# M2-TE/noetic-slam

Hardware: AMD Instinct MI355X
Metric: scans/sec TSDF integration (128x1024 pts, 5 cm voxel) (higher is better)
Workload: dtype f64+f32; 1 GPU; C1/M1 ouster_os1_128_1024x10_synthetic_5cm; global_batch=64, scans_per_gpu_batch=64, pipelined_batches=2, semantics=vdbfusion_f64, parallelism=single, front_end=two walks (k_count + k_place)

## Files before the change

noetic-slam_amd/csrc/tsdf_capi.cpp:

```cpp
#include <hip/hip_runtime.h>

#include <algorithm>
#include <array>
#include <atomic>
#include <cmath>
#include <cstdarg>
#include <cstddef>
#include <cstdio>
#include <cstdlib>
#include <cstring>
#include <numeric>
#include <chrono>
#include <condition_variable>
#include <functional>
#include <mutex>
#include <string>
#include <thread>
#include <utility>
#include <vector>

#include "../../include/tsdf_hip.h"
#include "../../include/tsdf_hip_deskew.h"
#include "../../include/tsdf_hip_columns.h"
#include "../../include/tsdf_hip_esdf.h"
// ... 181 lines not shown
    HipHandle() = default;
    HipHandle(const HipHandle&) = delete;
    HipHandle& operator=(const HipHandle&) = delete;
    ~HipHandle() { if (h) (void)KILL(h); }
    hipError_t create() { return MAKE(&h, FLAGS); }
    operator H() const { return h; }
};
using Event = HipHandle<hipEvent_t, hipEventCreateWithFlags, hipEventDisableTiming, hipEventDestroy>;
using Stream = HipHandle<hipStream_t, hipStreamCreateWithFlags, hipStreamNonBlocking, hipStreamDestroy>;


struct Capacity {
    uint64_t max_bricks = 0, cap = 0;
    uint32_t max_active = 0;
    DevBuf<uint64_t> keys, brick_keys;
    DevBuf<uint32_t> slots, touched, cell[2];
    DevBuf<float> sdf, weight;
    DevBuf<uint4> active[2], active_ord[2], cagg[2];
};

struct Lane {
    DevBuf<uint32_t> pair, blk_n, plan, spn, ord_hist, act;
    DevBuf<uint32_t> tile;
    DevBuf<uint4> blk, fb;
    DevBuf<uint2> smp;
    DevBuf<uint64_t> mg_ekey;
    DevBuf<uint32_t> mg_eidx, mg_bcnt, mg_bst, mg_bscan;
    DevBuf<float> mg_xyz, mg_w;
};

struct ScanRing {
    static constexpr int N = 16;
    PinBuf<ScanRec> host;
// ... 231 lines not shown
    if (lean) HIPCHK(c, hipEventRecord(c->ev_compact[par], st));
    if (prev && !lean) HIPCHK(c, hipStreamWaitEvent(st, c->ev_integ[par ^ 1], 0));
    if (D.n_blocks) {
        if (tm && c->plan.fused) tm->begin(KIND_INTEGRATE, st);
        if (small) {
            HIPCHK(c, launch_integrate_small(B, c->R, T, W, c->Pl, c->G, par, st, kt(KIND_INTEGRATE)));
        } else {
            Work Wi = W;
            Wi.active = W.active_ord;
            HIPCHK(c, launch_integrate(B, c->R, T, Wi, c->Pl, c->G, par, c->plan.fused, c->max_batch > 64, st,
                                       kt(KIND_INTEGRATE)));
        }
        if (tm && c->plan.fused) tm->end(KIND_INTEGRATE, st);
        c->ht.lap(HT_INTEGRATE);
    }
    HIPCHK(c, launch_finish(c->G, par, (uint32_t)c->batch_id, B, st));
    if (cross) {
        HIPCHK(c, hipEventRecord(ring.ev[slot], st));
        c->ev_integ[par] = ring.ev[slot];
    }
    if (c->can_grow) c->log.push_back({c->batch_id, d_xyz, D});
    for (int k = 0; k < 2; k++)
        if (d_xyz == c->stage2[k]) {
            c->stage_reader[k] = c->batch_id;
            HIPCHK(c, hipEventRecord(c->stage_ev[k], st));
        }
    c->ht.lap(HT_FINISH);
    c->ht.n++;
    c->batch_id++;
    c->n_batches++;
    c->n_scans += D.n_scans;
// ... 59 lines not shown

static int settle(tsdf_ctx* c) {
    const int rc = flush(c);
    return rc ? rc : join(c);
}


static int alloc_capacity(tsdf_ctx* c, uint64_t max_bricks, Capacity& K) {
    K = Capacity{};
    K.max_bricks = max_bricks;
    K.cap = next_pow2(2 * max_bricks);
    K.max_active = (uint32_t)std::min<uint64_t>(K.cap, c->plan.slots);
    const size_t cells = K.cap * c->plan.cell_stride * (c->plan.fused ? sizeof(uint64_t) : sizeof(uint32_t));
    hipError_t e = K.keys.alloc(K.cap);
    if (e == hipSuccess) e = K.slots.alloc(K.cap);
    if (e == hipSuccess) e = K.touched.alloc(K.cap);
    if (e == hipSuccess) e = K.brick_keys.alloc(max_bricks);
    if (e == hipSuccess) e = K.sdf.alloc(max_bricks * BRICK_VOX);
    if (e == hipSuccess) e = K.weight.alloc(max_bricks * BRICK_VOX);
    for (int q = 0; q < 2 && e == hipSuccess; q++) {
        e = K.cell[q].alloc_bytes(cells);
        if (e == hipSuccess) e = K.active[q].alloc(K.max_active);
        if (e == hipSuccess) e = K.active_ord[q].alloc(K.max_active);
        if (e == hipSuccess) e = K.cagg[q].alloc(compact_chunks(K.cap) * 2);
    }
    if (e != hipSuccess) {
        (void)hipGetLastError();
        return fail(c, TSDF_ENOMEM, "device allocation for %llu bricks failed",
                    (unsigned long long)max_bricks);
    }
    e = launch_fill_u64(K.keys, EMPTY_KEY, K.cap, c->stream);
    if (e == hipSuccess) e = launch_fill_u32(K.slots, UNASSIGNED, K.cap, c->stream);
    if (e == hipSuccess) e = hipMemsetAsync(K.touched, 0, K.cap * sizeof(uint32_t), c->stream);
    for (int q = 0; q < 2 && e == hipSuccess; q++) e = hipMemsetAsync(K.cell[q], 0, cells, c->stream);
    if (e != hipSuccess) return fail(c, TSDF_EHIP, "capacity init: %s", hipGetErrorString(e));
    return TSDF_OK;
}

static void set_views(tsdf_ctx* c) {
    const Capacity& K = c->K;
    c->T = Table{K.keys, K.slots, K.touched, K.cell[0], K.brick_keys, K.cap - 1,
                 (uint32_t)K.max_bricks, c->plan.cell_stride};
    c->Pl = Pool{K.sdf, K.weight};
    const uint64_t mg_cap = c->merged ? c->plan.batch_points : 0;
    for (int q = 0; q < 2; q++) {
        const Lane& L = c->lane[q];
        c->W2[q] = Work{L.pair, L.blk, L.blk_n, L.plan, L.fb, L.smp, K.active[q], K.active_ord[q],
                        L.ord_hist, K.cagg[q], L.act, L.spn, c->plan.maxp,
                        K.max_active, c->max_fb, c->max_smp, c->max_spn};
        c->mg[q] = MgBufs{L.mg_xyz, L.mg_w, mg_cap, L.mg_ekey, L.mg_eidx, L.mg_bcnt, L.mg_bst,
                          L.mg_bscan, mg_cap ? mg_buckets_max(mg_cap) : 0};
    }
}


struct GlobalsCheck { uint32_t pool_count, overflow, failed, retry, fail_id; };
static_assert(offsetof(Globals, pool_count) == 0 && offsetof(Globals, overflow) == 4 &&
              offsetof(Globals, failed) == 8 && offsetof(Globals, retry) == 12 &&
              offsetof(Globals, fail_id) == 16 && offsetof(Globals, ctr) < offsetof(Globals, tot_vox),
              "the host reads and clears Globals' head by these offsets");
static hipError_t globals_clear(uint32_t* first, int words) {
    const uint32_t z[3] = {0u, 0u, 0u};
    return hipMemcpy(first, z, 4 * words, hipMemcpyHostToDevice);
// ... 21 lines not shown
        if (e == hipSuccess)
            e = hipMemcpyAsync(K.brick_keys, c->T.brick_keys, valid * 8, hipMemcpyDeviceToDevice,
                               c->stream);
    }
    if (e == hipSuccess) e = launch_fill(K.sdf + valid * BRICK_VOX, c->R.bg, (nb - valid) * BRICK_VOX, c->stream);
    if (e == hipSuccess)
        e = hipMemsetAsync(K.weight + valid * BRICK_VOX, 0, (nb - valid) * BRICK_VOX * 4, c->stream);
    if (e == hipSuccess) e = hipStreamSynchronize(c->stream);
    if (e != hipSuccess) return fail(c, TSDF_EHIP, "grow: %s", hipGetErrorString(e));
    c->K = std::move(K);
    set_views(c);
    HIPCHK(c, launch_rehash(c->T, (uint32_t)valid, c->G, c->stream));
    const uint32_t pcv = (uint32_t)valid, retry = 1u;
    HIPCHK(c, hipMemsetAsync(c->G, 0, offsetof(Globals, tot_vox), c->stream));
    HIPCHK(c, hipMemcpyAsync(&c->G->pool_count, &pcv, 4, hipMemcpyHostToDevice, c->stream));
    HIPCHK(c, hipMemcpyAsync(&c->G->retry, &retry, 4, hipMemcpyHostToDevice, c->stream));
    HIPCHK(c, hipStreamSynchronize(c->stream));
    c->n_grows++;
    return TSDF_OK;
}

template <class T>
static int grow_list(tsdf_ctx* c, DevBuf<T> Lane::*list, uint32_t tsdf_ctx::*max, uint64_t limit,
                     size_t bytes, const char* what, bool counted) {
    const uint64_t n = std::min<uint64_t>(2ull * (c->*max), limit);
    if (n <= c->*max) return fail(c, TSDF_ENOMEM, "%s at its limit", what);
    DevBuf<T> f[2];
    hipError_t e = f[0].alloc_bytes(n * bytes);
    if (e == hipSuccess) e = f[1].alloc_bytes(n * bytes);
    if (e != hipSuccess) {
// ... 1740 lines not shown
            if (rc == TSDF_EHIP) return rc;
        }
    }
    Scratch tmp;
    int32_t* dc = nullptr;
    float *ds = nullptr, *dw = nullptr;
    uint32_t* dt = nullptr;
    HIPCHK(c, tmp.get(c, &dc, n * 3));
    HIPCHK(c, tmp.get(c, &ds, n * BRICK_VOX));
    HIPCHK(c, tmp.get(c, &dw, n * BRICK_VOX));
    HIPCHK(c, tmp.get(c, &dt, n));
    HIPCHK(c, hipMemcpyAsync(dc, coords, n * 12, hipMemcpyHostToDevice, c->stream));
    HIPCHK(c, hipMemcpyAsync(ds, sdf, n * BRICK_VOX * 4, hipMemcpyHostToDevice, c->stream));
    HIPCHK(c, hipMemcpyAsync(dw, weight, n * BRICK_VOX * 4, hipMemcpyHostToDevice, c->stream));
    HIPCHK(c, launch_import(c->T, c->Pl, dc, (uint32_t)n, ds, dw, dt, c->G, merge_cap(c), c->stream));
    HIPCHK(c, hipStreamSynchronize(c->stream));
    return tsdf_sync(c);
}

}


static int merge_ctx_state(tsdf_ctx* d, tsdf_ctx* c, const char* which) {
    if (c->p.n_sectors > 1)
        return fail(d, TSDF_EINVAL, "merge: the %s context holds one sector shard of the map "
                                    "(n_sectors > 1); merging a sharded field is not supported", which);
    if (c->brd_open)
        return fail(d, TSDF_EINVAL, "merge: a border reduce is open on the %s context: commit or "
                                    "abort it first (tsdf_border_commit_device)", which);
    return TSDF_OK;
// ... 73 lines not shown
    if (!apply || !st.touched_bricks) return TSDF_OK;

    const uint64_t need = n_dst + st.new_bricks;
    if (need > d->T.max_bricks) {
        if (!d->can_grow || (d->p.max_bricks_hard && need > d->p.max_bricks_hard) ||
            need > 0xFFFFFFEFull)
            return fail(d, TSDF_ENOMEM, "merge: %llu new bricks do not fit the pool (%llu of %llu "
                                        "bricks in use) and it cannot grow",
                        (unsigned long long)st.new_bricks, (unsigned long long)n_dst,
                        (unsigned long long)d->T.max_bricks);
        rc = grow_capacity(d, need);
        if (rc) return rc;
    }
    HIPCHK(d, launch_merge_apply(d->T, d->Pl, s->T, s->Pl, s->R, X, mode, min_weight, merge_cap(d),
                                 list, n_cand, flag, tslot, d->G, d->stream));
    HIPCHK(d, hipStreamSynchronize(d->stream));
    return tsdf_sync(d);
}

extern "C" {

int tsdf_merge_count(tsdf_ctx* dst, tsdf_ctx* src, const double pose[12], int32_t mode,
                     float min_weight, tsdf_merge_stats* out) {
    return merge_impl(dst, src, pose, mode, min_weight, out, false);
}

int tsdf_merge_transformed(tsdf_ctx* dst, tsdf_ctx* src, const double pose[12], int32_t mode,
                           float min_weight, tsdf_merge_stats* out) {
    return merge_impl(dst, src, pose, mode, min_weight, out, true);
}
// ... 32 lines not shown
                    M.new_count, M.n, M.n_moves);
    return TSDF_OK;
}

static int removal_compact(tsdf_ctx* c, const Removal& M) {
    if (!M.removed()) return TSDF_OK;
    const Capacity& K = c->K;
    const uint64_t at = (uint64_t)M.new_count * BRICK_VOX, freed = (uint64_t)M.removed() * BRICK_VOX;
    HIPCHK(c, launch_rm_move(c->T, c->Pl, M.rml, M.mover, M.n_moves, c->stream));
    HIPCHK(c, launch_fill(c->Pl.sdf + at, c->R.bg, freed, c->stream));
    HIPCHK(c, hipMemsetAsync(c->Pl.weight + at, 0, freed * sizeof(float), c->stream));
    HIPCHK(c, launch_fill_u64(K.keys, EMPTY_KEY, K.cap, c->stream));
    HIPCHK(c, launch_fill_u32(K.slots, UNASSIGNED, K.cap, c->stream));
    const size_t cells = K.cap * c->plan.cell_stride *
                         (c->plan.fused ? sizeof(uint64_t) : sizeof(uint32_t));
    HIPCHK(c, hipMemsetAsync(K.touched, 0, K.cap * sizeof(uint32_t), c->stream));
    for (int q = 0; q < 2; q++) HIPCHK(c, hipMemsetAsync(K.cell[q], 0, cells, c->stream));
    HIPCHK(c, launch_rehash(c->T, M.new_count, c->G, c->stream));
    HIPCHK(c, hipMemcpyAsync(&c->G->pool_count, &M.new_count, 4, hipMemcpyHostToDevice, c->stream));
    HIPCHK(c, hipStreamSynchronize(c->stream));
    return TSDF_OK;
}

static int removal_enter(tsdf_ctx* c, const int32_t* lo, const int32_t* hi, bool box, uint64_t* nb) {
    if (border_busy(c)) return TSDF_EINVAL;
    if (box) {
        if (!lo || !hi) return fail(c, TSDF_EINVAL, "null box");
        for (int a = 0; a < 3; a++)
            if (lo[a] > hi[a]) return fail(c, TSDF_EINVAL, "box: lo > hi");
    }
    return pool_bricks(c, nb);
}

extern "C" {
// ... 592 lines not shown
```

noetic-slam_amd/csrc/tsdf_device.h:

```cpp
#pragma once
#include <hip/hip_ext.h>
#include <hip/hip_runtime.h>
#include <stdint.h>

#include "os_headers.h"

namespace tsdf {

constexpr uint64_t EMPTY_KEY = ~0ull;
constexpr uint32_t UNASSIGNED = 0xFFFFFFFFu;
constexpr uint32_t INVALID_SLOT = 0xFFFFFFFEu;
constexpr uint32_t NO_PAIR = 0xFFFFFFFFu;
constexpr int BRICK_VOX = 512;
constexpr int BRICK_COORD_BIAS = 1 << 20;
constexpr int VOX_LIMIT = 1 << 23;
constexpr int MAX_DDA_STEPS = 1 << 20;
constexpr int MAX_BATCH = 512;
#ifndef TSDF_RPB
#define TSDF_RPB 1024
#endif
#ifndef TSDF_HCAP
#define TSDF_HCAP 2048
#endif
constexpr int RPB = TSDF_RPB;
// ... 76 lines not shown
struct BatchDesc {
    uint32_t n_scans;
    uint32_t n_blocks;
    ScanRec s[MAX_BATCH + 1];
};
struct BatchRef {
    uint32_t n_scans;
    uint32_t n_blocks;
    const ScanRec* __restrict__ s;
    const uint32_t* __restrict__ tile;
};

struct Table {
    uint64_t* keys;
    uint32_t* slots;
    uint32_t* touched;
    uint32_t* cell;
    uint64_t* brick_keys;
    uint64_t mask;
    uint32_t max_bricks;
    uint32_t cell_stride;
};

struct Pool {
    float* sdf;
    float* weight;
};

struct Work {
    uint32_t* pair;
    uint4* blk;
    uint32_t* blk_n;
    uint32_t* plan;
    uint4* fb;
    uint2* smp;
    uint4* active;
    uint4* active_ord;
    uint32_t* ord_hist;
    uint4* cagg;
    uint32_t* act;
    uint32_t* spn;
    uint32_t maxp;
    uint32_t max_active;
    uint32_t max_fb;
    uint32_t max_smp;
    uint32_t max_spn;
};

constexpr size_t smp_bytes(int sem) { return sem == 3 ? 12 : 8; }
template <int SEM>
__device__ __forceinline__ void smp_store(const Work& W, uint32_t i, float s, uint32_t tl, float w) {
    if constexpr (SEM == 3)
        reinterpret_cast<uint3*>(W.smp)[i] = make_uint3(__float_as_uint(s), tl, __float_as_uint(w));
    else
// ... 28 lines not shown
constexpr uint32_t METRIC_RING = 256;
struct BatchRecord {
    uint32_t batch_id, n_active, n_new, ovf;
    uint32_t committed, pool_count;
    uint32_t tiled;
    uint32_t pad;
    unsigned long long rays, pairs, vox, dirty;
};

struct Globals {
    uint32_t pool_count;
    uint32_t overflow;
    uint32_t failed;
    uint32_t retry;
    uint32_t fail_id;
    uint32_t pad[3];
    Counters ctr[2];
    unsigned long long tot_vox[8];
    unsigned long long tot_rays[8];
    unsigned long long tot_pairs[8];
    unsigned long long tot_dirty[8];
    Counters last;
    BatchRecord ring[METRIC_RING];
};

enum KernelKind {
    KIND_COUNT = 0, KIND_COMPACT = 1, KIND_PLACE = 2, KIND_INTEGRATE = 3,
    KIND_WALK = 4, KIND_SPANS = 5,
    KIND_N = 6
};

// ... 14 lines not shown
    virtual void begin(int kind, hipStream_t st) = 0;
    virtual void end(int kind, hipStream_t st) = 0;
    virtual ~KernelTimer() {}
};

hipError_t launch_count(const float* d_xyz, const BatchRef& D, const RayConst& R, const Table& T,
                        const Work& Wk, Globals* G, int parity, hipStream_t st, const KTime& kt = {},
                        bool wide = false, bool paired = false);
hipError_t launch_tile_detect(const float* d_xyz, const BatchRef& D, uint32_t* tile,
                              uint32_t force, hipStream_t st);
#ifndef TSDF_CMP_CHUNK
#define TSDF_CMP_CHUNK 1024
#endif
constexpr uint32_t CMP_CHUNK = TSDF_CMP_CHUNK;
inline uint64_t compact_chunks(uint64_t cap) { return (cap + CMP_CHUNK - 1) / CMP_CHUNK; }
hipError_t launch_sector_flags(const float* d_xyz, const BatchRef& D, const RayConst& R,
                               const Work& Wk, Globals* G, int parity, hipStream_t st);
hipError_t launch_compact(const BatchRef& D, const Table& T, const Work& Wk, Globals* G,
                          int parity, bool fused, hipStream_t st, const KTime& kt = {});
hipError_t launch_walk(const float* d_xyz, const BatchRef& D, const RayConst& R, const Table& T,
                       const Work& Wk, Globals* G, int parity, int nstep, hipStream_t st);
hipError_t launch_spans(const BatchRef& D, const RayConst& R, const Table& T, const Work& Wk,
                        Globals* G, int parity, int nstep, hipStream_t st);
hipError_t launch_place(const float* d_xyz, const BatchRef& D, const RayConst& R, const Table& T,
                        const Work& Wk, Globals* G, int parity, hipStream_t st, const KTime& kt = {});
hipError_t launch_finish(Globals* G, int parity, uint32_t batch_id, const BatchRef& D,
                         hipStream_t st);
hipError_t launch_pool_mark(Globals* G, int parity, hipStream_t st);
hipError_t launch_upload(const void* host_src, void* dst, uint32_t bytes,
                         unsigned long long* done, unsigned long long seq, hipStream_t st);
hipError_t launch_rehash(const Table& T, uint32_t n, Globals* G, hipStream_t st);
hipError_t launch_integrate_small(const BatchRef& D, const RayConst& R, const Table& T,
                                  const Work& Wk, const Pool& Pl, Globals* G, int parity,
                                  hipStream_t st, const KTime& kt = {});
hipError_t launch_integrate(const BatchRef& D, const RayConst& R, const Table& T, const Work& Wk,
                            const Pool& Pl, Globals* G, int parity, bool fused, bool big,
                            hipStream_t st, const KTime& kt = {});
hipError_t launch_query_dense(const Table& T, const Pool& Pl, const int64_t lo[3], const int dims[3],
                              float bg, float* d_sdf, float* d_w, hipStream_t st);
hipError_t launch_import(const Table& T, const Pool& Pl, const int32_t* d_coords, uint32_t n,
                         const float* d_sdf, const float* d_w, uint32_t* d_tidx, Globals* G,
                         float max_w, hipStream_t st);
hipError_t launch_fill(float* p, float v, uint64_t n, hipStream_t st);
// ... 127 lines not shown
```

noetic-slam_amd/csrc/tsdf_kernels.hip:

```cpp
#include <hip/hip_runtime.h>
#include <stdint.h>

#include <type_traits>

#include "tsdf_device.h"
#include "tsdf_ray.h"

namespace tsdf {


__device__ __forceinline__ uint32_t xcd_wedge(uint32_t p, uint32_t n, uint32_t G) {
    const uint32_t grp = 8u * G, g0 = p - p % grp;
    if (g0 + grp > n) return p;
    const uint32_t i = p - g0;
    return g0 + (i % 8u) * G + i / 8u;
}

__device__ __forceinline__ int lds_insert(unsigned long long* s_key, uint64_t key) {
    uint32_t hs = (uint32_t)(mix64(key) >> 40) & (HCAP - 1);
    for (int p = 0; p < LDS_PROBES; p++) {
        const unsigned long long k = s_key[hs];
        if (k == key) return (int)hs;
        if (k == EMPTY_KEY) {
            const unsigned long long old = atomicCAS(&s_key[hs], EMPTY_KEY, key);
// ... 454 lines not shown

constexpr int ORD_BLOCKS = 64;
constexpr int ORD_CLASSES = 32;

__device__ __forceinline__ uint32_t size_class(uint32_t n) {
    return (uint32_t)__clz(max(n, 1u));
}
__device__ __forceinline__ uint32_t ord_chunk_slice(uint32_t c, uint32_t nch) {
    return (uint32_t)(((uint64_t)c * ORD_BLOCKS) / nch);
}


constexpr int CMP_THREADS = 256;
constexpr int CMP_PER = CMP_CHUNK / CMP_THREADS;
constexpr int CMP_GROUP = 16;
constexpr int CMP_SCAN_THREADS = 1024;

template <int NT>
__device__ __forceinline__ uint32_t block_excl_scan(uint32_t x, uint32_t* s_w, uint32_t* total) {
    constexpr int NW = NT / 64;
    const int lane = threadIdx.x & 63, wid = threadIdx.x >> 6;
    const uint32_t v = wave_incl_scan(x);
    if (lane == 63) s_w[wid] = v;
    __syncthreads();
    uint32_t off = 0, tot = 0;
#pragma unroll
    for (int k = 0; k < NW; k++) {
        const uint32_t r = s_w[k];
        off += k < wid ? r : 0u;
        tot += r;
    }
    *total = tot;
    __syncthreads();
    return v - x + off;
}

__device__ __forceinline__ uint32_t compact_list(const Table& T, uint32_t chunk, uint32_t* s_h,
                                                 uint32_t* s_w, bool clear) {
    uint32_t hit[CMP_PER], cnt = 0;
#pragma unroll
    for (int j = 0; j < CMP_PER; j++) {
        const uint32_t h = chunk + threadIdx.x * CMP_PER + j;
        hit[j] = h <= T.mask && T.touched[h] != 0u ? 1u : 0u;
        cnt += hit[j];
    }
    uint32_t nh;
    uint32_t e = block_excl_scan<CMP_THREADS>(cnt, s_w, &nh);
#pragma unroll
    for (int j = 0; j < CMP_PER; j++) {
        if (hit[j]) {
            const uint32_t h = chunk + threadIdx.x * CMP_PER + j;
            s_h[e++] = h;
            if (clear) T.touched[h] = 0u;
        }
    }
    __syncthreads();
    return nh;
}

template <bool FUSED>
__device__ __forceinline__ uint32_t row_groups(uint32_t n_scans) {
    return FUSED ? (n_scans + 2) / 2 : (n_scans + 3) / 4;
}
template <bool FUSED>
__device__ __forceinline__ uint32_t group_count(const uint4& v) {
    return FUSED ? v.y + v.w : v.x + v.y + v.z + v.w;
}
template <bool FUSED>
__device__ __forceinline__ const uint4* cell_row(const Table& T, uint32_t h) {
// ... 1 lines not shown
                                                  (size_t)h * T.cell_stride)
                 : reinterpret_cast<const uint4*>(T.cell + (size_t)h * T.cell_stride);
}

template <bool FUSED>
__global__ __launch_bounds__(CMP_THREADS) void k_compact_sum(uint32_t n_scans, Table T, Work Wk) {
    __shared__ uint32_t s_w[CMP_THREADS / 64];
    __shared__ uint32_t s_h[CMP_CHUNK];
    __shared__ uint32_t s_acc[2];
    if (threadIdx.x == 0) {
        s_acc[0] = 0u;
        s_acc[1] = 0u;
    }
    __shared__ uint32_t s_cls[ORD_CLASSES];
    if (threadIdx.x < ORD_CLASSES) s_cls[threadIdx.x] = 0u;
    const uint32_t nh = compact_list(T, blockIdx.x * CMP_CHUNK, s_h, s_w, false);
    const uint32_t nq = row_groups<FUSED>(n_scans);
    const uint32_t grp = threadIdx.x / CMP_GROUP, li = threadIdx.x % CMP_GROUP;
    uint32_t samples = 0, nnew = 0;
    for (uint32_t k = grp; k < nh; k += CMP_THREADS / CMP_GROUP) {
        const uint32_t h = s_h[k];
        const uint4* cp = cell_row<FUSED>(T, h);
        uint32_t sum = 0;
        for (uint32_t q = li; q < nq; q += CMP_GROUP) sum += group_count<FUSED>(cp[q]);
        samples += sum;
#pragma unroll
        for (int d = CMP_GROUP / 2; d >= 1; d >>= 1) sum += __shfl_xor(sum, d, CMP_GROUP);
        if (li == 0) atomicAdd(&s_cls[size_class(sum)], 1u);
        if (li == 0 && T.slots[h] == UNASSIGNED) nnew++;
    }
    samples = wave_sum<uint32_t>(samples);
    nnew = wave_sum<uint32_t>(nnew);
    if ((threadIdx.x & 63) == 0) {
        if (samples) atomicAdd(&s_acc[0], samples);
        if (nnew) atomicAdd(&s_acc[1], nnew);
    }
    __syncthreads();
    if (threadIdx.x == 0) Wk.cagg[blockIdx.x] = make_uint4(nh, s_acc[0], s_acc[1], 0u);
    if (threadIdx.x < ORD_CLASSES && s_cls[threadIdx.x])
        atomicAdd(&Wk.ord_hist[ord_chunk_slice(blockIdx.x, gridDim.x) * ORD_CLASSES + threadIdx.x],
                  s_cls[threadIdx.x]);
}

__global__ __launch_bounds__(CMP_SCAN_THREADS) void k_compact_scan(uint32_t nch, Work Wk,
                                                                   Globals* G, int parity,
                                                                   int fused) {
    __shared__ uint32_t s_w[3][CMP_SCAN_THREADS / 64];
    __shared__ uint32_t s_carry[3];
    Counters* C = &G->ctr[parity];
    if (threadIdx.x == 0) {
        s_carry[0] = 0u;
        s_carry[1] = 0u;
        s_carry[2] = G->pool_count;
    }
    __syncthreads();
    constexpr int NWS = CMP_SCAN_THREADS / 64;
    const int lane = threadIdx.x & 63, wid = threadIdx.x >> 6;
    const uint32_t P = (nch + CMP_SCAN_THREADS - 1) / CMP_SCAN_THREADS;
    const uint32_t c0 = threadIdx.x * P;
    uint32_t sa = 0, sc = 0, sn = 0;
#pragma unroll 4
    for (uint32_t q = 0; q < P; q++) {
        const uint4 a = c0 + q < nch ? Wk.cagg[c0 + q] : make_uint4(0u, 0u, 0u, 0u);
        sa += a.x;
        sc += a.y;
        sn += a.z;
    }
    const uint32_t ia = wave_incl_scan(sa), ic = wave_incl_scan(sc), in = wave_incl_scan(sn);
    if (lane == 63) {
        s_w[0][wid] = ia;
        s_w[1][wid] = ic;
        s_w[2][wid] = in;
    }
    __syncthreads();
    uint32_t oa = s_carry[0], oc = s_carry[1], on = s_carry[2], ta = 0, tc = 0, tn = 0;
#pragma unroll
    for (int k = 0; k < NWS; k++) {
        const uint32_t xa = s_w[0][k], xc = s_w[1][k], xn = s_w[2][k];
        oa += k < wid ? xa : 0u;
        oc += k < wid ? xc : 0u;
        on += k < wid ? xn : 0u;
        ta += xa;
        tc += xc;
        tn += xn;
    }
    oa += ia - sa;
    oc += ic - sc;
    on += in - sn;
    for (uint32_t q = 0; q < P && c0 + q < nch; q++) {
        const uint4 a = Wk.cagg[c0 + q];
        Wk.cagg[nch + c0 + q] = make_uint4(oa, oc, on, 0u);
        oa += a.x;
        oc += a.y;
        on += a.z;
    }
    if (threadIdx.x == 0) {
        s_carry[0] += ta;
        s_carry[1] += tc;
        s_carry[2] += tn;
    }
    __syncthreads();
    static_assert(ORD_BLOCKS == 64 && ORD_CLASSES == 32 && CMP_SCAN_THREADS == 1024, "layout");
    {
        __shared__ uint32_t s_tot[ORD_CLASSES], s_cbase[ORD_CLASSES];
        const int lane = threadIdx.x & 63, w = threadIdx.x >> 6;
        uint32_t v[2], ex[2];
#pragma unroll
        for (int q = 0; q < 2; q++) {
            const int cls = w + 16 * q;
            v[q] = Wk.ord_hist[lane * ORD_CLASSES + cls];
            const uint32_t incl = wave_incl_scan(v[q]);
            ex[q] = incl - v[q];
            if (lane == 63) s_tot[cls] = incl;
            Wk.ord_hist[lane * ORD_CLASSES + cls] = 0u;
        }
        __syncthreads();
        if (w == 0) {
            const uint32_t t = lane < ORD_CLASSES ? s_tot[lane] : 0u;
            const uint32_t incl = wave_incl_scan(t);
            if (lane < ORD_CLASSES) s_cbase[lane] = incl - t;
        }
        __syncthreads();
#pragma unroll
        for (int q = 0; q < 2; q++) {
            const int cls = w + 16 * q;
            Wk.ord_hist[ORD_BLOCKS * ORD_CLASSES + lane * ORD_CLASSES + cls] = s_cbase[cls] + ex[q];
        }
    }
    if (threadIdx.x == 0) {
        C->n_active = s_carry[0];
        C->cursor = s_carry[1];
        C->n_new = s_carry[2] - G->pool_count;
        G->pool_count = s_carry[2];
        C->pool = s_carry[2];
        if (fused ? s_carry[1] > Wk.max_spn : s_carry[1] > Wk.max_smp)
            atomicOr(&C->ovf, fused ? OVF_SPN : OVF_SMP);
        if (s_carry[0] > Wk.max_active) atomicOr(&C->ovf, OVF_ACTIVE);
    }
}

template <bool FUSED>
__global__ __launch_bounds__(CMP_THREADS) void k_compact_write(uint32_t n_scans, uint32_t nch,
                                                               Table T, Work Wk, Globals* G,
                                                               int parity) {
    __shared__ uint32_t s_w[CMP_THREADS / 64];
    __shared__ uint32_t s_h[CMP_CHUNK];
    __shared__ uint32_t s_n[CMP_CHUNK];
    const uint32_t chunk = blockIdx.x * CMP_CHUNK;
    const uint32_t nh = compact_list(T, chunk, s_h, s_w, true);
    if (nh == 0) return;
    const uint32_t nq = row_groups<FUSED>(n_scans);
    const uint32_t grp = threadIdx.x / CMP_GROUP, li = threadIdx.x % CMP_GROUP;
    for (uint32_t k = grp; k < nh; k += CMP_THREADS / CMP_GROUP) {
        const uint4* cp = cell_row<FUSED>(T, s_h[k]);
        uint32_t sum = 0;
        for (uint32_t q = li; q < nq; q += CMP_GROUP) sum += group_count<FUSED>(cp[q]);
#pragma unroll
        for (int d = CMP_GROUP / 2; d >= 1; d >>= 1) sum += __shfl_xor(sum, d, CMP_GROUP);
        if (li == 0) s_n[k] = sum;
    }
    __syncthreads();
    const uint4 base = Wk.cagg[nch + blockIdx.x];
    uint32_t n[CMP_PER], isnew[CMP_PER], sn = 0, snew = 0;
#pragma unroll
    for (int j = 0; j < CMP_PER; j++) {
        const uint32_t k = threadIdx.x * CMP_PER + j;
        n[j] = k < nh ? s_n[k] : 0u;
        isnew[j] = k < nh && T.slots[s_h[k]] == UNASSIGNED ? 1u : 0u;
        sn += n[j];
        snew += isnew[j];
    }
    uint32_t tc, tn;
    uint32_t ec = block_excl_scan<CMP_THREADS>(sn, s_w, &tc);
    uint32_t en = block_excl_scan<CMP_THREADS>(snew, s_w, &tn);
#pragma unroll
    for (int j = 0; j < CMP_PER; j++) {
        const uint32_t k = threadIdx.x * CMP_PER + j;
        if (k < nh) {
            const uint32_t h = s_h[k];
            uint32_t slot = isnew[j] ? base.z + en : T.slots[h];
            if (isnew[j]) {
                if (slot < T.max_bricks) {
                    T.brick_keys[slot] = T.keys[h];
                } else {
                    slot = INVALID_SLOT;
                    atomicOr(&G->ctr[parity].ovf, OVF_POOL);
                }
                T.slots[h] = slot;
            }
            const uint4 rec = make_uint4(h, slot, base.y + ec, n[j]);
            if (base.x + k < Wk.max_active) Wk.active[base.x + k] = rec;
            const uint32_t op = atomicAdd(&Wk.ord_hist[ORD_BLOCKS * ORD_CLASSES +
                                                       ord_chunk_slice(blockIdx.x, gridDim.x) * ORD_CLASSES +
                                                       size_class(n[j])], 1u);
            if (op < Wk.max_active) Wk.active_ord[op] = rec;
            s_n[k] = base.y + ec;
        }
        ec += n[j];
        en += isnew[j];
    }
    __syncthreads();
    if constexpr (FUSED) {
        for (uint32_t k = grp; k < nh; k += CMP_THREADS / CMP_GROUP) {
            uint4* cp = const_cast<uint4*>(cell_row<true>(T, s_h[k]));
            uint32_t cs = 0, cp_ = s_n[k];
            for (uint32_t q0 = 0; q0 < nq; q0 += CMP_GROUP) {
                const uint32_t q = q0 + li;
                uint4 v = q < nq ? cp[q] : make_uint4(0u, 0u, 0u, 0u);
                const uint32_t s2 = v.x + v.z, p2 = v.y + v.w;
// ... 399 lines not shown
        constexpr int NT2 = 2 * CNT_THREADS;
        auto k = R.sem == 3 ? k_count<3, NT2, 2> : R.sem == 1 ? k_count<1, NT2, 2> : R.sem == 2 ? k_count<2, NT2, 2> : k_count<0, NT2, 2>;
        tlaunch(k, (D.n_blocks + 1) / 2, NT2, st, kt.start, kt.stop, d_xyz, D, R, T, Wk, G, parity);
    } else {
        auto k = R.sem == 3 ? k_count<3> : R.sem == 1 ? k_count<1> : R.sem == 2 ? k_count<2> : k_count<0>;
        tlaunch(k, D.n_blocks, CNT_THREADS, st, kt.start, kt.stop, d_xyz, D, R, T, Wk, G, parity);
    }
    return hipGetLastError();
}

hipError_t launch_compact(const BatchRef& D, const Table& T, const Work& Wk, Globals* G,
                          int parity, bool fused, hipStream_t st, const KTime& kt) {
    const uint32_t nch = (uint32_t)compact_chunks(T.mask + 1);
    tlaunch(fused ? k_compact_sum<true> : k_compact_sum<false>, nch, CMP_THREADS, st, kt.start,
            nullptr, D.n_scans, T, Wk);
    k_compact_scan<<<1, CMP_SCAN_THREADS, 0, st>>>(nch, Wk, G, parity, fused ? 1 : 0);
    tlaunch(fused ? k_compact_write<true> : k_compact_write<false>, nch, CMP_THREADS, st, nullptr,
            kt.stop, D.n_scans, nch, T, Wk, G, parity);
    return hipGetLastError();
}

hipError_t launch_place(const float* d_xyz, const BatchRef& D, const RayConst& R, const Table& T,
                        const Work& Wk, Globals* G, int parity, hipStream_t st, const KTime& kt) {
    auto k = R.sem == 1 ? k_place<1> : R.sem == 3 ? k_place<3> : R.sem == 2 ? k_place<2> : k_place<0>;
    tlaunch(k, 2 * D.n_blocks, PLC_THREADS, st, kt.start, kt.stop, d_xyz, D, R, T, Wk, G, parity);
    return hipGetLastError();
}

__global__ void k_finish(Globals* G, int parity, uint32_t batch_id,
                         const uint32_t* __restrict__ tile, uint32_t n_scans) {
    constexpr int NW = sizeof(Counters) / 4;
    Counters* C = &G->ctr[parity];
    const uint32_t ovf = C->ovf, failed = G->failed;
    uint32_t tiled = 0;
    if (tile)
        for (uint32_t j = threadIdx.x; j < n_scans; j += 64) tiled += tile[j] ? 1u : 0u;
    tiled = wave_sum<uint32_t>(tiled);
    const bool commit = !(G->retry && (ovf || failed));
    __syncthreads();
    if (threadIdx.x < 8 && commit) {
        const int k = threadIdx.x;
        G->tot_rays[k] += C->n_rays[k];
        G->tot_pairs[k] += C->n_pairs[k];
        G->tot_vox[k] += C->n_vox[k];
        G->tot_dirty[k] += C->n_dirty[k];
// ... 19 lines not shown
        for (int k = 0; k < 8; k++) {
            r.rays += C->n_rays[k];
            r.pairs += C->n_pairs[k];
            r.vox += C->n_vox[k];
            r.dirty += C->n_dirty[k];
        }
        G->ring[batch_id % METRIC_RING] = r;
    }
    __syncthreads();
    uint32_t* src = reinterpret_cast<uint32_t*>(C);
    uint32_t* dst = reinterpret_cast<uint32_t*>(&G->last);
    for (int j = threadIdx.x; j < NW; j += blockDim.x) {
        dst[j] = src[j];
        src[j] = 0u;
    }
}

__global__ void k_upload(const uint4* __restrict__ src, uint4* __restrict__ dst, uint32_t n,
                         unsigned long long* done, unsigned long long seq) {
    for (uint32_t i = threadIdx.x; i < n; i += blockDim.x) dst[i] = src[i];
    __syncthreads();
    if (threadIdx.x == 0)
        __hip_atomic_fetch_max(done, seq, __ATOMIC_RELEASE, __HIP_MEMORY_SCOPE_SYSTEM);
}

hipError_t launch_upload(const void* host_src, void* dst, uint32_t bytes,
                         unsigned long long* done, unsigned long long seq, hipStream_t st) {
    k_upload<<<1, 256, 0, st>>>(static_cast<const uint4*>(host_src), static_cast<uint4*>(dst),
                                bytes / 16, done, seq);
    return hipGetLastError();
}

__global__ void k_pool_mark(Globals* G, int parity) { G->ctr[parity].pool = G->pool_count; }

hipError_t launch_pool_mark(Globals* G, int parity, hipStream_t st) {
    k_pool_mark<<<1, 1, 0, st>>>(G, parity);
    return hipGetLastError();
}

hipError_t launch_finish(Globals* G, int parity, uint32_t batch_id, const BatchRef& D,
                         hipStream_t st) {
    k_finish<<<1, 64, 0, st>>>(G, parity, batch_id, D.tile, D.n_scans);
    return hipGetLastError();
}

__global__ void k_rehash(Table T, uint32_t n, Globals* G) {
    for (uint32_t slot = blockIdx.x * blockDim.x + threadIdx.x; slot < n;
         slot += gridDim.x * blockDim.x) {
        const int64_t h = table_insert(T, T.brick_keys[slot], &G->overflow);
        if (h >= 0) T.slots[h] = slot;
    }
}

hipError_t launch_rehash(const Table& T, uint32_t n, Globals* G, hipStream_t st) {
    if (n) k_rehash<<<grid_for(n, 256, 4096), 256, 0, st>>>(T, n, G);
    return hipGetLastError();
}
// ... 35 lines not shown
```

Before: 61100 scans/s.

## Drop single-block compact scan kernel; fold prefix sums into compact write

```diff
diff --git a/noetic-slam_amd/csrc/tsdf_capi.cpp b/noetic-slam_amd/csrc/tsdf_capi.cpp
--- a/noetic-slam_amd/csrc/tsdf_capi.cpp
+++ b/noetic-slam_amd/csrc/tsdf_capi.cpp
@@ -219,9 +219,12 @@
     uint64_t max_bricks = 0, cap = 0;
     uint32_t max_active = 0;
     DevBuf<uint64_t> keys, brick_keys;
-    DevBuf<uint32_t> slots, touched, cell[2];
+    DevBuf<uint32_t> slots, cell[2];
+    DevBuf<uint8_t> touched;
     DevBuf<float> sdf, weight;
     DevBuf<uint4> active[2], active_ord[2], cagg[2];
+    DevBuf<uint16_t> clist[2];
+    DevBuf<uint32_t> ctot[2];
 };
 
 struct Lane {
@@ -483,7 +486,7 @@
         if (tm && c->plan.fused) tm->end(KIND_INTEGRATE, st);
         c->ht.lap(HT_INTEGRATE);
     }
-    HIPCHK(c, launch_finish(c->G, par, (uint32_t)c->batch_id, B, st));
+    HIPCHK(c, launch_finish(c->G, par, (uint32_t)c->batch_id, B, W, st));
     if (cross) {
         HIPCHK(c, hipEventRecord(ring.ev[slot], st));
         c->ev_integ[par] = ring.ev[slot];
@@ -573,7 +576,7 @@
     const size_t cells = K.cap * c->plan.cell_stride * (c->plan.fused ? sizeof(uint64_t) : sizeof(uint32_t));
     hipError_t e = K.keys.alloc(K.cap);
     if (e == hipSuccess) e = K.slots.alloc(K.cap);
-    if (e == hipSuccess) e = K.touched.alloc(K.cap);
+    if (e == hipSuccess) e = K.touched.alloc(compact_entries(K.cap));
     if (e == hipSuccess) e = K.brick_keys.alloc(max_bricks);
     if (e == hipSuccess) e = K.sdf.alloc(max_bricks * BRICK_VOX);
     if (e == hipSuccess) e = K.weight.alloc(max_bricks * BRICK_VOX);
@@ -581,7 +584,9 @@
         e = K.cell[q].alloc_bytes(cells);
         if (e == hipSuccess) e = K.active[q].alloc(K.max_active);
         if (e == hipSuccess) e = K.active_ord[q].alloc(K.max_active);
-        if (e == hipSuccess) e = K.cagg[q].alloc(compact_chunks(K.cap) * 2);
+        if (e == hipSuccess) e = K.cagg[q].alloc(compact_chunks(K.cap));
+        if (e == hipSuccess) e = K.clist[q].alloc(compact_entries(K.cap));
+        if (e == hipSuccess) e = K.ctot[q].alloc(compact_entries(K.cap));
     }
     if (e != hipSuccess) {
         (void)hipGetLastError();
@@ -590,7 +595,7 @@
     }
     e = launch_fill_u64(K.keys, EMPTY_KEY, K.cap, c->stream);
     if (e == hipSuccess) e = launch_fill_u32(K.slots, UNASSIGNED, K.cap, c->stream);
-    if (e == hipSuccess) e = hipMemsetAsync(K.touched, 0, K.cap * sizeof(uint32_t), c->stream);
+    if (e == hipSuccess) e = hipMemsetAsync(K.touched, 0, compact_entries(K.cap), c->stream);
     for (int q = 0; q < 2 && e == hipSuccess; q++) e = hipMemsetAsync(K.cell[q], 0, cells, c->stream);
     if (e != hipSuccess) return fail(c, TSDF_EHIP, "capacity init: %s", hipGetErrorString(e));
     return TSDF_OK;
@@ -605,7 +610,7 @@
     for (int q = 0; q < 2; q++) {
         const Lane& L = c->lane[q];
         c->W2[q] = Work{L.pair, L.blk, L.blk_n, L.plan, L.fb, L.smp, K.active[q], K.active_ord[q],
-                        L.ord_hist, K.cagg[q], L.act, L.spn, c->plan.maxp,
+                        L.ord_hist, K.cagg[q], K.clist[q], K.ctot[q], L.act, L.spn, c->plan.maxp,
                         K.max_active, c->max_fb, c->max_smp, c->max_spn};
         c->mg[q] = MgBufs{L.mg_xyz, L.mg_w, mg_cap, L.mg_ekey, L.mg_eidx, L.mg_bcnt, L.mg_bst,
                           L.mg_bscan, mg_cap ? mg_buckets_max(mg_cap) : 0};
@@ -657,6 +662,7 @@
     const uint32_t pcv = (uint32_t)valid, retry = 1u;
     HIPCHK(c, hipMemsetAsync(c->G, 0, offsetof(Globals, tot_vox), c->stream));
     HIPCHK(c, hipMemcpyAsync(&c->G->pool_count, &pcv, 4, hipMemcpyHostToDevice, c->stream));
+    HIPCHK(c, launch_pool_sync(c->G, c->stream));
     HIPCHK(c, hipMemcpyAsync(&c->G->retry, &retry, 4, hipMemcpyHostToDevice, c->stream));
     HIPCHK(c, hipStreamSynchronize(c->stream));
     c->n_grows++;
@@ -2427,6 +2433,7 @@
     HIPCHK(c, hipMemcpyAsync(ds, sdf, n * BRICK_VOX * 4, hipMemcpyHostToDevice, c->stream));
     HIPCHK(c, hipMemcpyAsync(dw, weight, n * BRICK_VOX * 4, hipMemcpyHostToDevice, c->stream));
     HIPCHK(c, launch_import(c->T, c->Pl, dc, (uint32_t)n, ds, dw, dt, c->G, merge_cap(c), c->stream));
+    HIPCHK(c, launch_pool_sync(c->G, c->stream));
     HIPCHK(c, hipStreamSynchronize(c->stream));
     return tsdf_sync(c);
 }
@@ -2530,6 +2537,7 @@
     }
     HIPCHK(d, launch_merge_apply(d->T, d->Pl, s->T, s->Pl, s->R, X, mode, min_weight, merge_cap(d),
                                  list, n_cand, flag, tslot, d->G, d->stream));
+    HIPCHK(d, launch_pool_sync(d->G, d->stream));
     HIPCHK(d, hipStreamSynchronize(d->stream));
     return tsdf_sync(d);
 }
@@ -2592,10 +2600,11 @@
     HIPCHK(c, launch_fill_u32(K.slots, UNASSIGNED, K.cap, c->stream));
     const size_t cells = K.cap * c->plan.cell_stride *
                          (c->plan.fused ? sizeof(uint64_t) : sizeof(uint32_t));
-    HIPCHK(c, hipMemsetAsync(K.touched, 0, K.cap * sizeof(uint32_t), c->stream));
+    HIPCHK(c, hipMemsetAsync(K.touched, 0, compact_entries(K.cap), c->stream));
     for (int q = 0; q < 2; q++) HIPCHK(c, hipMemsetAsync(K.cell[q], 0, cells, c->stream));
     HIPCHK(c, launch_rehash(c->T, M.new_count, c->G, c->stream));
     HIPCHK(c, hipMemcpyAsync(&c->G->pool_count, &M.new_count, 4, hipMemcpyHostToDevice, c->stream));
+    HIPCHK(c, launch_pool_sync(c->G, c->stream));
     HIPCHK(c, hipStreamSynchronize(c->stream));
     return TSDF_OK;
 }
diff --git a/noetic-slam_amd/csrc/tsdf_device.h b/noetic-slam_amd/csrc/tsdf_device.h
--- a/noetic-slam_amd/csrc/tsdf_device.h
+++ b/noetic-slam_amd/csrc/tsdf_device.h
@@ -114,7 +114,7 @@
 struct Table {
     uint64_t* keys;
     uint32_t* slots;
-    uint32_t* touched;
+    uint8_t* touched;
     uint32_t* cell;
     uint64_t* brick_keys;
     uint64_t mask;
@@ -138,6 +138,8 @@
     uint4* active_ord;
     uint32_t* ord_hist;
     uint4* cagg;
+    uint16_t* clist;
+    uint32_t* ctot;
     uint32_t* act;
     uint32_t* spn;
     uint32_t maxp;
@@ -196,7 +198,8 @@
     uint32_t failed;
     uint32_t retry;
     uint32_t fail_id;
-    uint32_t pad[3];
+    uint32_t pool_par[2];
+    uint32_t pad;
     Counters ctr[2];
     unsigned long long tot_vox[8];
     unsigned long long tot_rays[8];
@@ -241,6 +244,7 @@
 #endif
 constexpr uint32_t CMP_CHUNK = TSDF_CMP_CHUNK;
 inline uint64_t compact_chunks(uint64_t cap) { return (cap + CMP_CHUNK - 1) / CMP_CHUNK; }
+inline uint64_t compact_entries(uint64_t cap) { return compact_chunks(cap) * CMP_CHUNK; }
 hipError_t launch_sector_flags(const float* d_xyz, const BatchRef& D, const RayConst& R,
                                const Work& Wk, Globals* G, int parity, hipStream_t st);
 hipError_t launch_compact(const BatchRef& D, const Table& T, const Work& Wk, Globals* G,
@@ -252,8 +256,9 @@
 hipError_t launch_place(const float* d_xyz, const BatchRef& D, const RayConst& R, const Table& T,
                         const Work& Wk, Globals* G, int parity, hipStream_t st, const KTime& kt = {});
 hipError_t launch_finish(Globals* G, int parity, uint32_t batch_id, const BatchRef& D,
-                         hipStream_t st);
+                         const Work& Wk, hipStream_t st);
 hipError_t launch_pool_mark(Globals* G, int parity, hipStream_t st);
+hipError_t launch_pool_sync(Globals* G, hipStream_t st);
 hipError_t launch_upload(const void* host_src, void* dst, uint32_t bytes,
                          unsigned long long* done, unsigned long long seq, hipStream_t st);
 hipError_t launch_rehash(const Table& T, uint32_t n, Globals* G, hipStream_t st);
diff --git a/noetic-slam_amd/csrc/tsdf_kernels.hip b/noetic-slam_amd/csrc/tsdf_kernels.hip
--- a/noetic-slam_amd/csrc/tsdf_kernels.hip
+++ b/noetic-slam_amd/csrc/tsdf_kernels.hip
@@ -492,7 +492,6 @@
 constexpr int CMP_THREADS = 256;
 constexpr int CMP_PER = CMP_CHUNK / CMP_THREADS;
 constexpr int CMP_GROUP = 16;
-constexpr int CMP_SCAN_THREADS = 1024;
 
 template <int NT>
 __device__ __forceinline__ uint32_t block_excl_scan(uint32_t x, uint32_t* s_w, uint32_t* total) {
@@ -514,23 +513,26 @@
 }
 
 __device__ __forceinline__ uint32_t compact_list(const Table& T, uint32_t chunk, uint32_t* s_h,
-                                                 uint32_t* s_w, bool clear) {
-    uint32_t hit[CMP_PER], cnt = 0;
-#pragma unroll
-    for (int j = 0; j < CMP_PER; j++) {
-        const uint32_t h = chunk + threadIdx.x * CMP_PER + j;
-        hit[j] = h <= T.mask && T.touched[h] != 0u ? 1u : 0u;
-        cnt += hit[j];
+                                                 uint32_t* s_w) {
+    static_assert(CMP_PER % 4 == 0, "a thread's touched flags are whole u32 words");
+    const uint32_t h0 = chunk + threadIdx.x * CMP_PER;
+    uint32_t* fw = reinterpret_cast<uint32_t*>(T.touched + h0);
+    uint32_t w[CMP_PER / 4], cnt = 0;
+#pragma unroll
+    for (int q = 0; q < CMP_PER / 4; q++) {
+        w[q] = fw[q];
+#pragma unroll
+        for (int j = 0; j < 4; j++) cnt += (w[q] >> (8 * j)) & 0xffu ? 1u : 0u;
     }
     uint32_t nh;
     uint32_t e = block_excl_scan<CMP_THREADS>(cnt, s_w, &nh);
 #pragma unroll
-    for (int j = 0; j < CMP_PER; j++) {
-        if (hit[j]) {
-            const uint32_t h = chunk + threadIdx.x * CMP_PER + j;
-            s_h[e++] = h;
-            if (clear) T.touched[h] = 0u;
-        }
+    for (int q = 0; q < CMP_PER / 4; q++) {
+        if (w[q] == 0u) continue;
+#pragma unroll
+        for (int j = 0; j < 4; j++)
+            if ((w[q] >> (8 * j)) & 0xffu) s_h[e++] = h0 + 4 * q + j;
+        fw[q] = 0u;
     }
     __syncthreads();
     return nh;
@@ -562,7 +564,11 @@
     }
     __shared__ uint32_t s_cls[ORD_CLASSES];
     if (threadIdx.x < ORD_CLASSES) s_cls[threadIdx.x] = 0u;
-    const uint32_t nh = compact_list(T, blockIdx.x * CMP_CHUNK, s_h, s_w, false);
+    const uint32_t chunk = blockIdx.x * CMP_CHUNK;
+    const uint32_t nh = compact_list(T, chunk, s_h, s_w);
+    uint16_t* lst = Wk.clist + (size_t)chunk;
+    uint32_t* tot = Wk.ctot + (size_t)chunk;
+    for (uint32_t k = threadIdx.x; k < nh; k += CMP_THREADS) lst[k] = (uint16_t)(s_h[k] - chunk);
     const uint32_t nq = row_groups<FUSED>(n_scans);
     const uint32_t grp = threadIdx.x / CMP_GROUP, li = threadIdx.x % CMP_GROUP;
     uint32_t samples = 0, nnew = 0;
@@ -574,8 +580,11 @@
         samples += sum;
 #pragma unroll
         for (int d = CMP_GROUP / 2; d >= 1; d >>= 1) sum += __shfl_xor(sum, d, CMP_GROUP);
-        if (li == 0) atomicAdd(&s_cls[size_class(sum)], 1u);
-        if (li == 0 && T.slots[h] == UNASSIGNED) nnew++;
+        if (li == 0) {
+            tot[k] = sum;
+            atomicAdd(&s_cls[size_class(sum)], 1u);
+            if (T.slots[h] == UNASSIGNED) nnew++;
+        }
     }
     samples = wave_sum<uint32_t>(samples);
     nnew = wave_sum<uint32_t>(nnew);
@@ -590,133 +599,113 @@
                   s_cls[threadIdx.x]);
 }
 
-__global__ __launch_bounds__(CMP_SCAN_THREADS) void k_compact_scan(uint32_t nch, Work Wk,
-                                                                   Globals* G, int parity,
-                                                                   int fused) {
-    __shared__ uint32_t s_w[3][CMP_SCAN_THREADS / 64];
-    __shared__ uint32_t s_carry[3];
-    Counters* C = &G->ctr[parity];
-    if (threadIdx.x == 0) {
-        s_carry[0] = 0u;
-        s_carry[1] = 0u;
-        s_carry[2] = G->pool_count;
-    }
-    __syncthreads();
-    constexpr int NWS = CMP_SCAN_THREADS / 64;
-    const int lane = threadIdx.x & 63, wid = threadIdx.x >> 6;
-    const uint32_t P = (nch + CMP_SCAN_THREADS - 1) / CMP_SCAN_THREADS;
-    const uint32_t c0 = threadIdx.x * P;
-    uint32_t sa = 0, sc = 0, sn = 0;
-#pragma unroll 4
-    for (uint32_t q = 0; q < P; q++) {
-        const uint4 a = c0 + q < nch ? Wk.cagg[c0 + q] : make_uint4(0u, 0u, 0u, 0u);
-        sa += a.x;
-        sc += a.y;
-        sn += a.z;
-    }
-    const uint32_t ia = wave_incl_scan(sa), ic = wave_incl_scan(sc), in = wave_incl_scan(sn);
-    if (lane == 63) {
-        s_w[0][wid] = ia;
-        s_w[1][wid] = ic;
-        s_w[2][wid] = in;
-    }
-    __syncthreads();
-    uint32_t oa = s_carry[0], oc = s_carry[1], on = s_carry[2], ta = 0, tc = 0, tn = 0;
-#pragma unroll
-    for (int k = 0; k < NWS; k++) {
-        const uint32_t xa = s_w[0][k], xc = s_w[1][k], xn = s_w[2][k];
-        oa += k < wid ? xa : 0u;
-        oc += k < wid ? xc : 0u;
-        on += k < wid ? xn : 0u;
-        ta += xa;
-        tc += xc;
-        tn += xn;
-    }
-    oa += ia - sa;
-    oc += ic - sc;
-    on += in - sn;
-    for (uint32_t q = 0; q < P && c0 + q < nch; q++) {
-        const uint4 a = Wk.cagg[c0 + q];
-        Wk.cagg[nch + c0 + q] = make_uint4(oa, oc, on, 0u);
-        oa += a.x;
-        oc += a.y;
-        on += a.z;
-    }
-    if (threadIdx.x == 0) {
-        s_carry[0] += ta;
-        s_carry[1] += tc;
-        s_carry[2] += tn;
-    }
-    __syncthreads();
-    static_assert(ORD_BLOCKS == 64 && ORD_CLASSES == 32 && CMP_SCAN_THREADS == 1024, "layout");
-    {
-        __shared__ uint32_t s_tot[ORD_CLASSES], s_cbase[ORD_CLASSES];
-        const int lane = threadIdx.x & 63, w = threadIdx.x >> 6;
-        uint32_t v[2], ex[2];
-#pragma unroll
-        for (int q = 0; q < 2; q++) {
-            const int cls = w + 16 * q;
-            v[q] = Wk.ord_hist[lane * ORD_CLASSES + cls];
-            const uint32_t incl = wave_incl_scan(v[q]);
-            ex[q] = incl - v[q];
-            if (lane == 63) s_tot[cls] = incl;
-            Wk.ord_hist[lane * ORD_CLASSES + cls] = 0u;
-        }
-        __syncthreads();
-        if (w == 0) {
-            const uint32_t t = lane < ORD_CLASSES ? s_tot[lane] : 0u;
-            const uint32_t incl = wave_incl_scan(t);
-            if (lane < ORD_CLASSES) s_cbase[lane] = incl - t;
-        }
-        __syncthreads();
-#pragma unroll
-        for (int q = 0; q < 2; q++) {
-            const int cls = w + 16 * q;
-            Wk.ord_hist[ORD_BLOCKS * ORD_CLASSES + lane * ORD_CLASSES + cls] = s_cbase[cls] + ex[q];
-        }
-    }
-    if (threadIdx.x == 0) {
-        C->n_active = s_carry[0];
-        C->cursor = s_carry[1];
-        C->n_new = s_carry[2] - G->pool_count;
-        G->pool_count = s_carry[2];
-        C->pool = s_carry[2];
-        if (fused ? s_carry[1] > Wk.max_spn : s_carry[1] > Wk.max_smp)
-            atomicOr(&C->ovf, fused ? OVF_SPN : OVF_SMP);
-        if (s_carry[0] > Wk.max_active) atomicOr(&C->ovf, OVF_ACTIVE);
-    }
+__device__ __forceinline__ uint32_t wave_total(uint32_t x) {
+    return (uint32_t)__builtin_amdgcn_readlane((int)wave_incl_scan(x), 63);
 }
 
 template <bool FUSED>
 __global__ __launch_bounds__(CMP_THREADS) void k_compact_write(uint32_t n_scans, uint32_t nch,
                                                                Table T, Work Wk, Globals* G,
                                                                int parity) {
-    __shared__ uint32_t s_w[CMP_THREADS / 64];
+    constexpr int NW = CMP_THREADS / 64;
+    __shared__ uint32_t s_w[NW];
     __shared__ uint32_t s_h[CMP_CHUNK];
     __shared__ uint32_t s_n[CMP_CHUNK];
+    __shared__ uint32_t s_pre[3][NW];
+    __shared__ uint32_t s_tot[ORD_CLASSES], s_pos[ORD_CLASSES];
     const uint32_t chunk = blockIdx.x * CMP_CHUNK;
-    const uint32_t nh = compact_list(T, chunk, s_h, s_w, true);
+    const uint4 mine = Wk.cagg[blockIdx.x];
+    const uint32_t nh = mine.x;
+    const bool last = blockIdx.x == nch - 1;
+    if (nh == 0 && !last) return;
+    const int lane = threadIdx.x & 63, wid = threadIdx.x >> 6;
+    {
+        uint32_t pa = 0, pc = 0, pn = 0;
+        for (uint32_t c = threadIdx.x; c < blockIdx.x; c += CMP_THREADS) {
+            const uint4 a = Wk.cagg[c];
+            pa += a.x;
+            pc += a.y;
+            pn += a.z;
+        }
+        pa = wave_total(pa);
+        pc = wave_total(pc);
+        pn = wave_total(pn);
+        if (lane == 0) {
+            s_pre[0][wid] = pa;
+            s_pre[1][wid] = pc;
+            s_pre[2][wid] = pn;
+        }
+    }
+    static_assert(ORD_BLOCKS == 64 && ORD_CLASSES == 8 * NW, "layout");
+    const uint32_t slice = ord_chunk_slice(blockIdx.x, nch);
+    {
+        const uint4* hp = reinterpret_cast<const uint4*>(Wk.ord_hist + lane * ORD_CLASSES + wid * 8);
+        const uint4 h0 = hp[0], h1 = hp[1];
+        const uint32_t v[8] = {h0.x, h0.y, h0.z, h0.w, h1.x, h1.y, h1.z, h1.w};
+#pragma unroll
+        for (int q = 0; q < 8; q++) {
+            const int incl = (int)wave_incl_scan(v[q]);
+            const uint32_t all = (uint32_t)__builtin_amdgcn_readlane(incl, 63);
+            const uint32_t before = slice ? (uint32_t)__builtin_amdgcn_readlane(incl, (int)slice - 1) : 0u;
+            if (lane == 0) {
+                s_tot[wid * 8 + q] = all;
+                s_pos[wid * 8 + q] = before;
+            }
+        }
+    }
+    __syncthreads();
+    if (wid == 0) {
+        const uint32_t t = lane < ORD_CLASSES ? s_tot[lane] : 0u;
+        const uint32_t incl = wave_incl_scan(t);
+        if (lane < ORD_CLASSES) s_pos[lane] += incl - t;
+    }
+    const uint32_t pool0 = G->pool_par[parity ^ 1];
+    uint4 base = make_uint4(0u, 0u, pool0, 0u);
+#pragma unroll
+    for (int k = 0; k < NW; k++) {
+        base.x += s_pre[0][k];
+        base.y += s_pre[1][k];
+        base.z += s_pre[2][k];
+    }
+    if (last && threadIdx.x == 0) {
+        Counters* C = &G->ctr[parity];
+        const uint32_t n_active = base.x + mine.x, cursor = base.y + mine.y, pool = base.z + mine.z;
+        C->n_active = n_active;
+        C->cursor = cursor;
+        C->n_new = pool - pool0;
+        C->pool = pool;
+        G->pool_par[parity] = pool;
+        G->pool_count = pool;
+        if (FUSED ? cursor > Wk.max_spn : cursor > Wk.max_smp) atomicOr(&C->ovf, FUSED ? OVF_SPN : OVF_SMP);
+        if (n_active > Wk.max_active) atomicOr(&C->ovf, OVF_ACTIVE);
+    }
     if (nh == 0) return;
     const uint32_t nq = row_groups<FUSED>(n_scans);
     const uint32_t grp = threadIdx.x / CMP_GROUP, li = threadIdx.x % CMP_GROUP;
-    for (uint32_t k = grp; k < nh; k += CMP_THREADS / CMP_GROUP) {
-        const uint4* cp = cell_row<FUSED>(T, s_h[k]);
-        uint32_t sum = 0;
-        for (uint32_t q = li; q < nq; q += CMP_GROUP) sum += group_count<FUSED>(cp[q]);
-#pragma unroll
-        for (int d = CMP_GROUP / 2; d >= 1; d >>= 1) sum += __shfl_xor(sum, d, CMP_GROUP);
-        if (li == 0) s_n[k] = sum;
-    }
-    __syncthreads();
-    const uint4 base = Wk.cagg[nch + blockIdx.x];
-    uint32_t n[CMP_PER], isnew[CMP_PER], sn = 0, snew = 0;
-#pragma unroll
-    for (int j = 0; j < CMP_PER; j++) {
-        const uint32_t k = threadIdx.x * CMP_PER + j;
-        n[j] = k < nh ? s_n[k] : 0u;
-        isnew[j] = k < nh && T.slots[s_h[k]] == UNASSIGNED ? 1u : 0u;
-        sn += n[j];
-        snew += isnew[j];
+    uint32_t n[CMP_PER], isnew[CMP_PER], hs[CMP_PER], slots[CMP_PER], sn = 0, snew = 0;
+#pragma unroll
+    for (int q = 0; q < CMP_PER / 4; q++) {
+        const uint32_t k0 = threadIdx.x * CMP_PER + 4 * q;
+        uint4 tv = make_uint4(0u, 0u, 0u, 0u);
+        uint2 lv = make_uint2(0u, 0u);
+        if (k0 < nh) {
+            tv = *reinterpret_cast<const uint4*>(Wk.ctot + (size_t)chunk + k0);
+            lv = *reinterpret_cast<const uint2*>(Wk.clist + (size_t)chunk + k0);
+        }
+        const uint32_t t4[4] = {tv.x, tv.y, tv.z, tv.w};
+        const uint32_t l4[4] = {lv.x & 0xffffu, lv.x >> 16, lv.y & 0xffffu, lv.y >> 16};
+#pragma unroll
+        for (int i = 0; i < 4; i++) {
+            const int j = 4 * q + i;
+            const bool in = k0 + i < nh;
+            hs[j] = chunk + l4[i];
+            n[j] = in ? t4[i] : 0u;
+            slots[j] = in ? T.slots[hs[j]] : 0u;
+            isnew[j] = in && slots[j] == UNASSIGNED ? 1u : 0u;
+            if (in) s_h[k0 + i] = hs[j];
+            sn += n[j];
+            snew += isnew[j];
+        }
     }
     uint32_t tc, tn;
     uint32_t ec = block_excl_scan<CMP_THREADS>(sn, s_w, &tc);
@@ -725,8 +714,8 @@
     for (int j = 0; j < CMP_PER; j++) {
         const uint32_t k = threadIdx.x * CMP_PER + j;
         if (k < nh) {
-            const uint32_t h = s_h[k];
-            uint32_t slot = isnew[j] ? base.z + en : T.slots[h];
+            const uint32_t h = hs[j];
+            uint32_t slot = isnew[j] ? base.z + en : slots[j];
             if (isnew[j]) {
                 if (slot < T.max_bricks) {
                     T.brick_keys[slot] = T.keys[h];
@@ -738,9 +727,9 @@
             }
             const uint4 rec = make_uint4(h, slot, base.y + ec, n[j]);
             if (base.x + k < Wk.max_active) Wk.active[base.x + k] = rec;
-            const uint32_t op = atomicAdd(&Wk.ord_hist[ORD_BLOCKS * ORD_CLASSES +
-                                                       ord_chunk_slice(blockIdx.x, gridDim.x) * ORD_CLASSES +
-                                                       size_class(n[j])], 1u);
+            const uint32_t cls = size_class(n[j]);
+            const uint32_t op = s_pos[cls] + atomicAdd(&Wk.ord_hist[ORD_BLOCKS * ORD_CLASSES +
+                                                                    slice * ORD_CLASSES + cls], 1u);
             if (op < Wk.max_active) Wk.active_ord[op] = rec;
             s_n[k] = base.y + ec;
         }
@@ -1170,7 +1159,6 @@
     const uint32_t nch = (uint32_t)compact_chunks(T.mask + 1);
     tlaunch(fused ? k_compact_sum<true> : k_compact_sum<false>, nch, CMP_THREADS, st, kt.start,
             nullptr, D.n_scans, T, Wk);
-    k_compact_scan<<<1, CMP_SCAN_THREADS, 0, st>>>(nch, Wk, G, parity, fused ? 1 : 0);
     tlaunch(fused ? k_compact_write<true> : k_compact_write<false>, nch, CMP_THREADS, st, nullptr,
             kt.stop, D.n_scans, nch, T, Wk, G, parity);
     return hipGetLastError();
@@ -1184,7 +1172,7 @@
 }
 
 __global__ void k_finish(Globals* G, int parity, uint32_t batch_id,
-                         const uint32_t* __restrict__ tile, uint32_t n_scans) {
+                         const uint32_t* __restrict__ tile, uint32_t n_scans, uint4* ord_hist) {
     constexpr int NW = sizeof(Counters) / 4;
     Counters* C = &G->ctr[parity];
     const uint32_t ovf = C->ovf, failed = G->failed;
@@ -1234,6 +1222,8 @@
         dst[j] = src[j];
         src[j] = 0u;
     }
+    for (int j = threadIdx.x; j < 2 * ORD_BLOCKS * ORD_CLASSES / 4; j += blockDim.x)
+        ord_hist[j] = make_uint4(0u, 0u, 0u, 0u);
 }
 
 __global__ void k_upload(const uint4* __restrict__ src, uint4* __restrict__ dst, uint32_t n,
@@ -1251,16 +1241,28 @@
     return hipGetLastError();
 }
 
-__global__ void k_pool_mark(Globals* G, int parity) { G->ctr[parity].pool = G->pool_count; }
+__global__ void k_pool_mark(Globals* G, int parity) {
+    const uint32_t pool = G->pool_par[parity ^ 1];
+    G->pool_par[parity] = pool;
+    G->ctr[parity].pool = pool;
+}
 
 hipError_t launch_pool_mark(Globals* G, int parity, hipStream_t st) {
     k_pool_mark<<<1, 1, 0, st>>>(G, parity);
     return hipGetLastError();
 }
 
+__global__ void k_pool_sync(Globals* G) { G->pool_par[0] = G->pool_par[1] = G->pool_count; }
+
+hipError_t launch_pool_sync(Globals* G, hipStream_t st) {
+    k_pool_sync<<<1, 1, 0, st>>>(G);
+    return hipGetLastError();
+}
+
 hipError_t launch_finish(Globals* G, int parity, uint32_t batch_id, const BatchRef& D,
-                         hipStream_t st) {
-    k_finish<<<1, 64, 0, st>>>(G, parity, batch_id, D.tile, D.n_scans);
+                         const Work& Wk, hipStream_t st) {
+    k_finish<<<1, 64, 0, st>>>(G, parity, batch_id, D.tile, D.n_scans,
+                               reinterpret_cast<uint4*>(Wk.ord_hist));
     return hipGetLastError();
 }
 
```

Measured after the change: 61560 scans/s, median of 6. No clear change (+0.8%).
